# AsherBond/0-kno-vectorx

Hardware: AMD Instinct MI355X
Metric: header_range_256 proofs/sec (higher is better)
Workload: dtype u64 (Goldilocks) / u8 (hashes)

## Files before the change

### 0-kno-vectorx_amd/csrc/poseidon.cuh

```cuda
#pragma once
#include <utility>
#include "gl.cuh"
#include "poseidon_constants.h"

static __constant__ uint64_t POSEIDON_RC[360] = VX_POSEIDON_RC_FOLDED_INIT;

__device__ __forceinline__ uint64_t poseidon_sbox(uint64_t x) {
    const uint64_t x2 = gl_mul_nc(x, x), x3 = gl_mul_nc(x2, x), x4 = gl_mul_nc(x2, x2);
    return gl_mul_nc(x3, x4);
}

template <class T, class TIn>
__device__ __forceinline__ void poseidon_mds_part(const TIn* x, T* y) {
    T u0[3], u2[3], ur[3], ui[3];
#pragma unroll
    for (int a = 0; a < 3; ++a) {
        const T x0 = (T)x[a], x1 = (T)x[3 + a], x2 = (T)x[6 + a], x3 = (T)x[9 + a];
        const T A = x0 + x2, B = x1 + x3;
        u0[a] = A + B;
        u2[a] = A - B;
        ur[a] = x0 - x2;
        ui[a] = x3 - x1;
    }
    const T s0 = u0[0] + u0[1] + u0[2];
    const T a0[3] = {s0 + u0[2], s0 + u0[0], s0 + u0[1]};
    const T a2[3] = {-u2[0] - 2 * u2[1] + 8 * u2[2], -8 * u2[0] - u2[1] - 2 * u2[2], 2 * u2[0] - 8 * u2[1] - u2[2]};
    T p0r[3], p0i[3], p1r[3], p1i[3], p2r[3], p2i[3];
#pragma unroll
    for (int a = 0; a < 3; ++a) {
        p0r[a] = 2 * ur[a] + ui[a];
        p0i[a] = 2 * ui[a] - ur[a];
        p1r[a] = -4 * ur[a] - ui[a];
        p1i[a] = ur[a] - 4 * ui[a];
        p2r[a] = 16 * ur[a] - ui[a];
        p2i[a] = 16 * ui[a] + ur[a];
    }
    const T r0 = p0r[0] + p2i[1] + p1i[2], i0 = p0i[0] - p2r[1] - p1r[2];
    const T r1 = p1r[0] + p0r[1] + p2i[2], i1 = p1i[0] + p0i[1] - p2r[2];
    const T r2 = p2r[0] + p1r[1] + p0r[2], i2 = p2i[0] + p1i[1] + p0i[2];
    const T rr[3] = {r0, r1, r2}, ii[3] = {i0, i1, i2};
#pragma unroll
    for (int c = 0; c < 3; ++c) {
        const T t = 16 * a0[c], pp = t + a2[c], mm = t - a2[c];
        y[c] = pp + rr[c];
        y[3 + c] = mm - ii[c];
        y[6 + c] = pp - rr[c];
        y[9 + c] = mm + ii[c];
    }
}

#ifndef VX_POSEIDON_FP64
#define VX_POSEIDON_FP64 0
#endif
#if VX_POSEIDON_FP64
struct PoseidonRcSplit {
    uint64_t d[360];
    uint32_t h[360];
};
constexpr PoseidonRcSplit poseidon_rc_split() {
    constexpr uint64_t rc[360] = VX_POSEIDON_RC_FOLDED_INIT;
    PoseidonRcSplit t{};
    for (int i = 0; i < 360; ++i) {
        t.d[i] = 0x4330000000000000ULL + (rc[i] & ((1ULL << 43) - 1));
        t.h[i] = (uint32_t)(rc[i] >> 43);
    }
    return t;
}
static __constant__ PoseidonRcSplit POSEIDON_RCT = poseidon_rc_split();
template <int RC>
__device__ __forceinline__ void poseidon_mds(uint64_t* s, int rc_next) {
    constexpr double TWO52 = 4503599627370496.0;
    double xl[12];
    uint32_t xh[12];
#pragma unroll
    for (int i = 0; i < 12; ++i) {
        const uint32_t lo = (uint32_t)s[i], hi = (uint32_t)(s[i] >> 32);
        xl[i] = __longlong_as_double((long long)(((uint64_t)(0x43300000u | (hi & 0x7FFu)) << 32) | lo)) - TWO52;
        xh[i] = hi >> 11;
    }
    double yl[12];
    int32_t yh[12];
    poseidon_mds_part<double>(xl, yl);
    poseidon_mds_part<int32_t>(xh, yh);
    yl[0] += xl[0] * (double)VX_POSEIDON_MDS_DIAG0;
    yh[0] += (int32_t)(xh[0] * VX_POSEIDON_MDS_DIAG0);
#pragma unroll
    for (int r = 0; r < 12; ++r) {
        double magic = TWO52;
        uint32_t ah = (uint32_t)yh[r];
        if (RC == 12 || (RC == 1 && r == 0)) {
            magic = __longlong_as_double((long long)POSEIDON_RCT.d[rc_next + r]);
            ah += POSEIDON_RCT.h[rc_next + r];
        }
        const uint64_t al = (uint64_t)__double_as_longlong(yl[r] + magic) & ((1ULL << 52) - 1);
        const uint64_t w = (uint64_t)(ah >> 21) * GL_EPS + al;
        uint32_t yhi;
        const bool carry = __builtin_add_overflow((uint32_t)(w >> 32), ah << 11, &yhi);
        const uint64_t y = ((uint64_t)yhi << 32) | (uint32_t)w;
        s[r] = y + (carry ? (uint64_t)GL_EPS : 0);
    }
}
#else
template <int RC>
__device__ __forceinline__ void poseidon_mds(uint64_t* s, int rc_next) {
    constexpr uint64_t M52 = (1ULL << 52) - 1;
    uint64_t xl[12];
    uint32_t xh[12];
#pragma unroll
    for (int i = 0; i < 12; ++i) {
        xl[i] = s[i] & M52;
        xh[i] = (uint32_t)(s[i] >> 52);
    }
    int64_t yl[12];
    int32_t yh[12];
    poseidon_mds_part<int64_t>(xl, yl);
    poseidon_mds_part<int32_t>(xh, yh);
    yl[0] += (int64_t)(xl[0] * VX_POSEIDON_MDS_DIAG0);
    yh[0] += (int32_t)(xh[0] * VX_POSEIDON_MDS_DIAG0);
#pragma unroll
    for (int r = 0; r < 12; ++r) {
        uint64_t al = (uint64_t)yl[r];
        uint32_t ah = (uint32_t)yh[r];
        if (RC == 12 || (RC == 1 && r == 0)) {
            const uint64_t c = POSEIDON_RC[rc_next + r];
            al += c & M52;
            ah += (uint32_t)(c >> 52);
        }
        const uint64_t w = (uint64_t)(ah >> 12) * GL_EPS + al;
        uint32_t yhi;
        const bool carry = __builtin_add_overflow((uint32_t)(w >> 32), ah << 20, &yhi);
        const uint64_t y = ((uint64_t)yhi << 32) | (uint32_t)w;
        s[r] = y + (carry ? (uint64_t)GL_EPS : 0);
    }
}

#endif

#ifndef VX_POSEIDON_SPLIT_PARTIAL
#define VX_POSEIDON_SPLIT_PARTIAL 1
#endif
__device__ __forceinline__ uint64_t poseidon_mds_split(uint64_t s0, uint64_t* xl, uint32_t* xh, int rc_next) {
    constexpr uint64_t M52 = (1ULL << 52) - 1;
    xl[0] = s0 & M52;
    xh[0] = (uint32_t)(s0 >> 52);
    int64_t yl[12];
    int32_t yh[12];
    poseidon_mds_part<int64_t>(xl, yl);
    poseidon_mds_part<int32_t>(xh, yh);
    yl[0] += (int64_t)(xl[0] * VX_POSEIDON_MDS_DIAG0);
    yh[0] += (int32_t)(xh[0] * VX_POSEIDON_MDS_DIAG0);
#pragma unroll
    for (int r = 1; r < 12; ++r) {
        const uint64_t al = (uint64_t)yl[r];
        const uint32_t hh = (uint32_t)yh[r] + (uint32_t)(al >> 52);
        xh[r] = hh & 0xFFFu;
        xl[r] = (uint64_t)(hh >> 12) * GL_EPS + (al & M52);
    }
    const uint64_t c = POSEIDON_RC[rc_next];
    const uint64_t al = (uint64_t)yl[0] + (c & M52);
    const uint32_t ah = (uint32_t)yh[0] + (uint32_t)(c >> 52);
    const uint64_t w = (uint64_t)(ah >> 12) * GL_EPS + al;
    uint32_t yhi;
    const bool carry = __builtin_add_overflow((uint32_t)(w >> 32), ah << 20, &yhi);
    const uint64_t y = ((uint64_t)yhi << 32) | (uint32_t)w;
    return y + (carry ? (uint64_t)GL_EPS : 0);
}
__device__ __forceinline__ void poseidon_mds_split_out(uint64_t s0, uint64_t* xl, uint32_t* xh, uint64_t* s, int rc_next) {
    constexpr uint64_t M52 = (1ULL << 52) - 1;
    xl[0] = s0 & M52;
    xh[0] = (uint32_t)(s0 >> 52);
    int64_t yl[12];
    int32_t yh[12];
    poseidon_mds_part<int64_t>(xl, yl);
    poseidon_mds_part<int32_t>(xh, yh);
    yl[0] += (int64_t)(xl[0] * VX_POSEIDON_MDS_DIAG0);
    yh[0] += (int32_t)(xh[0] * VX_POSEIDON_MDS_DIAG0);
#pragma unroll
    for (int r = 0; r < 12; ++r) {
        const uint64_t c = POSEIDON_RC[rc_next + r];
        const uint64_t al = (uint64_t)yl[r] + (c & M52);
        const uint32_t ah = (uint32_t)yh[r] + (uint32_t)(c >> 52);
        const uint64_t w = (uint64_t)(ah >> 12) * GL_EPS + al;
        uint32_t yhi;
        const bool carry = __builtin_add_overflow((uint32_t)(w >> 32), ah << 20, &yhi);
        const uint64_t y = ((uint64_t)yhi << 32) | (uint32_t)w;
        s[r] = y + (carry ? (uint64_t)GL_EPS : 0);
    }
}

template <bool CANON = true>
__device__ __forceinline__ void poseidon_permute(uint64_t* s) {
    int rc = 12;
#pragma unroll
    for (int i = 0; i < 12; ++i) s[i] = gl_add_nc(s[i], POSEIDON_RC[i]);
#pragma unroll 1
    for (int r = 0; r < 3; ++r) {
#pragma unroll
        for (int i = 0; i < 12; ++i) s[i] = poseidon_sbox(s[i]);
        poseidon_mds<12>(s, rc);
        rc += 12;
    }
#pragma unroll
    for (int i = 0; i < 12; ++i) s[i] = poseidon_sbox(s[i]);
    poseidon_mds<1>(s, rc);
    rc += 12;
#if VX_POSEIDON_SPLIT_PARTIAL && !VX_POSEIDON_FP64
    {
        constexpr uint64_t M52 = (1ULL << 52) - 1;
        uint64_t xl[12];
        uint32_t xh[12];
#pragma unroll
        for (int i = 1; i < 12; ++i) {
            xl[i] = s[i] & M52;
            xh[i] = (uint32_t)(s[i] >> 52);
        }
        uint64_t s0 = s[0];
#pragma unroll 1
        for (int r = 0; r < 21; ++r) {
            s0 = poseidon_mds_split(poseidon_sbox(s0), xl, xh, rc);
            rc += 12;
        }
        poseidon_mds_split_out(poseidon_sbox(s0), xl, xh, s, rc);
        rc += 12;
    }
#else
#pragma unroll 1
    for (int r = 0; r < 21; ++r) {
        s[0] = poseidon_sbox(s[0]);
        poseidon_mds<1>(s, rc);
        rc += 12;
    }
    s[0] = poseidon_sbox(s[0]);
    poseidon_mds<12>(s, rc);
    rc += 12;
#endif
#pragma unroll 1
    for (int r = 0; r < 3; ++r) {
#pragma unroll
        for (int i = 0; i < 12; ++i) s[i] = poseidon_sbox(s[i]);
        poseidon_mds<12>(s, rc);
        rc += 12;
    }
#pragma unroll
    for (int i = 0; i < 12; ++i) s[i] = poseidon_sbox(s[i]);
    poseidon_mds<0>(s, 0);
    if (CANON) {
#pragma unroll
        for (int i = 0; i < 12; ++i) s[i] = gl_canon(s[i]);
    }
}

__device__ __forceinline__ uint64_t poseidon_mds_coop(uint64_t s, int l, uint64_t* g) {
    constexpr uint32_t C[12] = VX_POSEIDON_MDS_CIRC_INIT;
    if (l < 12) g[l] = s;
    __builtin_amdgcn_fence(__ATOMIC_RELEASE, "wavefront");
    __builtin_amdgcn_wave_barrier();
    __builtin_amdgcn_fence(__ATOMIC_ACQUIRE, "wavefront");
    uint64_t al = 0, ah = 0;
    const int r = l < 12 ? l : 0;
#pragma unroll
    for (int i = 0; i < 12; ++i) {
        int j = r + i;
        if (j >= 12) j -= 12;
        const uint64_t x = g[j];
        al += (uint64_t)(uint32_t)x * C[i];
        ah += (x >> 32) * C[i];
    }
    if (l == 0) {
        const uint64_t x0 = g[0];
        al += (uint64_t)(uint32_t)x0 * VX_POSEIDON_MDS_DIAG0;
        ah += (x0 >> 32) * VX_POSEIDON_MDS_DIAG0;
    }
    __builtin_amdgcn_fence(__ATOMIC_RELEASE, "wavefront");
    __builtin_amdgcn_wave_barrier();
    __builtin_amdgcn_fence(__ATOMIC_ACQUIRE, "wavefront");
    const uint64_t w = (ah >> 32) * GL_EPS + al;
    uint32_t yhi;
    const bool carry = __builtin_add_overflow((uint32_t)(w >> 32), (uint32_t)ah, &yhi);
    const uint64_t y = ((uint64_t)yhi << 32) | (uint32_t)w;
    return y + (carry ? (uint64_t)GL_EPS : 0);
}
#ifndef VX_POSEIDON_COOP_DPP
#define VX_POSEIDON_COOP_DPP 1
#endif
template <int N>
__device__ __forceinline__ uint32_t dpp_ror(uint32_t x) {
    return (uint32_t)__builtin_amdgcn_update_dpp(0, (int)x, 0x120 + N, 0xf, 0xf, false);
}
struct CoopCoef {
    uint32_t c[16];
};
static __device__ const uint32_t POSEIDON_MDS_CIRC_DEV[12] = VX_POSEIDON_MDS_CIRC_INIT;
template <int N>
__device__ __forceinline__ void coop_coef_one(CoopCoef& k, int l) {
    const int q = (int)dpp_ror<N>((uint32_t)l);
    int d = q - l;
    if (d < 0) d += 12;
    k.c[N] = (q < 12 && l < 12) ? POSEIDON_MDS_CIRC_DEV[d < 12 ? d : 0] : 0;
}
template <int... Ns>
__device__ __forceinline__ void coop_coef_all(CoopCoef& k, int l, std::integer_sequence<int, Ns...>) {
    (coop_coef_one<Ns + 1>(k, l), ...);
}
template <int N>
__device__ __forceinline__ void coop_mac_one(const CoopCoef& k, uint64_t s, uint64_t& al, uint64_t& ah) {
    const uint32_t lo = dpp_ror<N>((uint32_t)s), hi = dpp_ror<N>((uint32_t)(s >> 32));
    al += (uint64_t)lo * k.c[N];
    ah += (uint64_t)hi * k.c[N];
}
template <int... Ns>
__device__ __forceinline__ void coop_mac_all(const CoopCoef& k, uint64_t s, uint64_t& al, uint64_t& ah, std::integer_sequence<int, Ns...>) {
    (coop_mac_one<Ns + 1>(k, s, al, ah), ...);
}
__device__ __forceinline__ uint64_t poseidon_mds_coop_dpp(uint64_t s, int l, const CoopCoef& k) {
    uint64_t al = (uint64_t)(uint32_t)s * k.c[0], ah = (s >> 32) * k.c[0];
    coop_mac_all(k, s, al, ah, std::make_integer_sequence<int, 15>{});
    if (l == 0) {
        al += (uint64_t)(uint32_t)s * VX_POSEIDON_MDS_DIAG0;
        ah += (s >> 32) * VX_POSEIDON_MDS_DIAG0;
    }
    const uint64_t w = (ah >> 32) * GL_EPS + al;
    uint32_t yhi;
    const bool carry = __builtin_add_overflow((uint32_t)(w >> 32), (uint32_t)ah, &yhi);
    const uint64_t y = ((uint64_t)yhi << 32) | (uint32_t)w;
    return y + (carry ? (uint64_t)GL_EPS : 0);
}
template <bool CANON = true>
__device__ __forceinline__ uint64_t poseidon_permute_coop(uint64_t s, int l, uint64_t* g) {
    const int lc = l < 12 ? l : 0;
#if VX_POSEIDON_COOP_DPP
    CoopCoef k;
    k.c[0] = l < 12 ? POSEIDON_MDS_CIRC_DEV[0] : 0;
    coop_coef_all(k, l, std::make_integer_sequence<int, 15>{});
    if (l >= 12) s = 0;
#pragma unroll 1
    for (int r = 0; r < 30; ++r) {
        s = gl_add_nc(s, POSEIDON_RC[12 * r + lc]);
        const bool full = r < 4 || r >= 26;
        if (full || l == 0) s = poseidon_sbox(s);
        s = poseidon_mds_coop_dpp(s, l, k);
    }
    return CANON ? gl_canon(s) : s;
#endif
#pragma unroll 1
    for (int r = 0; r < 30; ++r) {
        s = gl_add_nc(s, POSEIDON_RC[12 * r + lc]);
        const bool full = r < 4 || r >= 26;
        if (full || l == 0) s = poseidon_sbox(s);
        s = poseidon_mds_coop(s, l, g);
    }
    return CANON ? gl_canon(s) : s;
}
```

Measured before the change: 9.035.

## Keep Poseidon partial-round state in frequency domain across rounds

Replaces the 22 partial Poseidon rounds with a version that holds the 12-element state in a transformed (FFT-like) split 48/16-bit integer representation. Each round computes only the new element 0 and updates the transformed state incrementally, normalising lazily, with a single transform on entry and exit. This aims to cut the per-round MDS cost. In exchange it adds complex bound-dependent arithmetic that can overflow if the bounds are wrong, plus extra register pressure. It is enabled by default through a macro.

After: 9.508, median of 6. 1.05x the previous value.

```diff
diff --git a/0-kno-vectorx_amd/csrc/poseidon.cuh b/0-kno-vectorx_amd/csrc/poseidon.cuh
--- a/0-kno-vectorx_amd/csrc/poseidon.cuh
+++ b/0-kno-vectorx_amd/csrc/poseidon.cuh
@@ -188,20 +188,35 @@
     }
 }
 
-template <bool CANON = true>
-__device__ __forceinline__ void poseidon_permute(uint64_t* s) {
-    int rc = 12;
-#pragma unroll
-    for (int i = 0; i < 12; ++i) s[i] = gl_add_nc(s[i], POSEIDON_RC[i]);
-#pragma unroll 1
-    for (int r = 0; r < 3; ++r) {
-#pragma unroll
-        for (int i = 0; i < 12; ++i) s[i] = poseidon_sbox(s[i]);
-        poseidon_mds<12>(s, rc);
-        rc += 12;
-    }
-#pragma unroll
-    for (int i = 0; i < 12; ++i) s[i] = poseidon_sbox(s[i]);
+#ifndef VX_POSEIDON_FREQ_PARTIAL
+#define VX_POSEIDON_FREQ_PARTIAL 1
+#endif
+#if VX_POSEIDON_FREQ_PARTIAL
+#include "poseidon_freq.h"
+__device__ __forceinline__ void poseidon_partial_freq(uint64_t* s, int rc) {
+    pfreq::State u;
+    pfreq::enter(s, u);
+    uint64_t x0 = s[0];
+#pragma unroll 1
+    for (int r = 0; r < 11; ++r) {
+        uint64_t y0 = pfreq::round_y0(u, x0);
+        uint64_t t = poseidon_sbox(gl_add_nc(y0, POSEIDON_RC[rc]));
+        pfreq::round_put<false>(u, x0, y0, t);
+        x0 = t;
+        y0 = pfreq::round_y0(u, x0);
+        t = poseidon_sbox(gl_add_nc(y0, POSEIDON_RC[rc + 12]));
+        pfreq::round_put<true>(u, x0, y0, t);
+        x0 = t;
+        rc += 24;
+    }
+    pfreq::leave(u, x0, &POSEIDON_RC[rc], s);
+}
+#endif
+
+__device__ __forceinline__ void poseidon_partial_rounds(uint64_t* s, int rc) {
+#if VX_POSEIDON_FREQ_PARTIAL
+    poseidon_partial_freq(s, rc);
+#else
     poseidon_mds<1>(s, rc);
     rc += 12;
 #if VX_POSEIDON_SPLIT_PARTIAL && !VX_POSEIDON_FP64
@@ -221,7 +236,6 @@
             rc += 12;
         }
         poseidon_mds_split_out(poseidon_sbox(s0), xl, xh, s, rc);
-        rc += 12;
     }
 #else
 #pragma unroll 1
@@ -232,8 +246,26 @@
     }
     s[0] = poseidon_sbox(s[0]);
     poseidon_mds<12>(s, rc);
-    rc += 12;
-#endif
+#endif
+#endif
+}
+
+template <bool CANON = true>
+__device__ __forceinline__ void poseidon_permute(uint64_t* s) {
+    int rc = 12;
+#pragma unroll
+    for (int i = 0; i < 12; ++i) s[i] = gl_add_nc(s[i], POSEIDON_RC[i]);
+#pragma unroll 1
+    for (int r = 0; r < 3; ++r) {
+#pragma unroll
+        for (int i = 0; i < 12; ++i) s[i] = poseidon_sbox(s[i]);
+        poseidon_mds<12>(s, rc);
+        rc += 12;
+    }
+#pragma unroll
+    for (int i = 0; i < 12; ++i) s[i] = poseidon_sbox(s[i]);
+    poseidon_partial_rounds(s, rc);
+    rc += 12 * 23;
 #pragma unroll 1
     for (int r = 0; r < 3; ++r) {
 #pragma unroll
diff --git a/0-kno-vectorx_amd/csrc/poseidon_freq.h b/0-kno-vectorx_amd/csrc/poseidon_freq.h
--- /dev/null
+++ b/0-kno-vectorx_amd/csrc/poseidon_freq.h
@@ -0,0 +1,172 @@
+#pragma once
+#include <stdint.h>
+
+#if defined(__HIP_DEVICE_COMPILE__)
+#define PFREQ_FN __device__ __forceinline__
+#elif defined(__HIPCC__)
+#define PFREQ_FN __host__ __device__ inline
+#else
+#define PFREQ_FN static inline
+#endif
+#if defined(__clang__)
+#define PFREQ_UNROLL _Pragma("unroll")
+#else
+#define PFREQ_UNROLL
+#endif
+
+namespace pfreq {
+
+constexpr int LB = 48, HB = 16;
+constexpr uint64_t ML = (1ULL << LB) - 1;
+constexpr uint64_t EPS = 0xFFFFFFFFULL;
+constexpr uint64_t KL = (ML + 1 - EPS) << 12;
+constexpr uint32_t KH = ((1u << HB) - 1) << 12;
+constexpr int64_t BOUND_L = 4322LL << LB;
+constexpr int32_t BOUND_H = 4322 << HB;
+constexpr int64_t BOUND_YL = 3307LL << LB;
+constexpr int32_t BOUND_YH = 3307 << HB;
+
+struct State {
+    int64_t l[12];
+    int32_t h[12];
+};
+
+PFREQ_FN void keep(int64_t& x) {
+#if defined(__HIP_DEVICE_COMPILE__)
+    asm("" : "+v"(x));
+#else
+    (void)x;
+#endif
+}
+PFREQ_FN void keep(int32_t&) {}
+PFREQ_FN int32_t minus_one() {
+    int32_t k = -1;
+#if defined(__HIP_DEVICE_COMPILE__)
+    asm("" : "+s"(k));
+#endif
+    return k;
+}
+
+template <class T, class TIn>
+PFREQ_FN void fft_in(const TIn* x, T* u) {
+PFREQ_UNROLL
+    for (int a = 0; a < 3; ++a) {
+        const T x0 = (T)x[a], x1 = (T)x[3 + a], x2 = (T)x[6 + a], x3 = (T)x[9 + a];
+        const T A = x0 + x2, B = x1 + x3;
+        u[a] = A + B;
+        u[3 + a] = A - B;
+        u[6 + a] = x0 - x2;
+        u[9 + a] = x3 - x1;
+    }
+}
+
+template <class T>
+PFREQ_FN void block(const T* u, T* a) {
+    const T *u0 = u, *u2 = u + 3, *ur = u + 6, *ui = u + 9;
+    const T s0 = u0[0] + u0[1] + u0[2];
+    a[0] = s0 + u0[2], a[1] = s0 + u0[0], a[2] = s0 + u0[1];
+    T P, N;
+#define PFREQ_PN(i, pos, neg) P = pos, N = neg, keep(P), keep(N), a[i] = P - N, keep(a[i])
+    PFREQ_PN(3, 8 * u2[2], 2 * u2[1] + u2[0]);
+    PFREQ_PN(4, 0, 8 * u2[0] + 2 * u2[2] + u2[1]);
+    PFREQ_PN(5, 2 * u2[0], 8 * u2[1] + u2[2]);
+    PFREQ_PN(6, 16 * ui[1] + 2 * ur[0] + ui[0] + ur[1] + ur[2], 4 * ui[2]);
+    PFREQ_PN(9, 4 * ur[2] + 2 * ui[0] + ui[1] + ui[2], 16 * ur[1] + ur[0]);
+    PFREQ_PN(7, 16 * ui[2] + 2 * ur[1] + ui[1] + ur[2], 4 * ur[0] + ui[0]);
+    PFREQ_PN(10, 2 * ui[1] + ur[0] + ui[2], 16 * ur[2] + 4 * ui[0] + ur[1]);
+    PFREQ_PN(8, 16 * ur[0] + 2 * ur[2] + ui[2], 4 * ur[1] + ui[0] + ui[1]);
+    PFREQ_PN(11, 16 * ui[0] + 2 * ui[2] + ur[0] + ur[1], 4 * ui[1] + ur[2]);
+#undef PFREQ_PN
+    keep(a[0]), keep(a[1]), keep(a[2]);
+}
+
+PFREQ_FN uint64_t join(uint64_t l, uint32_t h) {
+    const uint64_t w = (uint64_t)(h >> HB) * EPS + l;
+    uint32_t yhi;
+    const bool carry = __builtin_add_overflow((uint32_t)(w >> 32), h << (32 - HB), &yhi);
+    const uint64_t y = ((uint64_t)yhi << 32) | (uint32_t)w;
+    return y + (carry ? EPS : 0);
+}
+
+PFREQ_FN void normalise(int64_t& l, int32_t& h) {
+    const int32_t hh = h + (int32_t)(l >> LB);
+    const int32_t u = hh >> HB;
+    h = hh & (int32_t)((1u << HB) - 1);
+    const uint32_t mhi = ((uint32_t)((uint64_t)l >> 32) & (uint32_t)(ML >> 32)) + (uint32_t)u;
+    l = (int64_t)(((uint64_t)mhi << 32) | (uint32_t)l) + (int64_t)u * (int64_t)minus_one();
+}
+
+PFREQ_FN void enter(const uint64_t* s, State& u) {
+    uint64_t xl[12];
+    uint32_t xh[12];
+PFREQ_UNROLL
+    for (int i = 0; i < 12; ++i) {
+        xl[i] = s[i] & ML;
+        xh[i] = (uint32_t)(s[i] >> LB);
+    }
+    fft_in<int64_t>(xl, u.l);
+    fft_in<int32_t>(xh, u.h);
+}
+
+PFREQ_FN uint64_t round_y0(State& u, uint64_t x0) {
+    int64_t al[12];
+    int32_t ah[12];
+    block<int64_t>(u.l, al);
+    block<int32_t>(u.h, ah);
+    const int64_t yl = 16 * al[0] + al[3] + al[6] + 8 * (int64_t)(x0 & ML);
+    const int32_t yh = 16 * ah[0] + ah[3] + ah[6] + 8 * (int32_t)(x0 >> LB);
+#ifdef PFREQ_TRACK_Y
+    PFREQ_TRACK_Y(yl, yh);
+#endif
+PFREQ_UNROLL
+    for (int c = 0; c < 3; ++c) {
+        u.l[c] = 64 * al[c], u.h[c] = 64 * ah[c];
+        u.l[3 + c] = 4 * al[3 + c], u.h[3 + c] = 4 * ah[3 + c];
+        u.l[6 + c] = 2 * al[6 + c], u.h[6 + c] = 2 * ah[6 + c];
+        u.l[9 + c] = 2 * al[9 + c], u.h[9 + c] = 2 * ah[9 + c];
+    }
+    return join((uint64_t)yl + KL, (uint32_t)yh + KH);
+}
+template <bool ALL>
+PFREQ_FN void round_put(State& u, uint64_t x0, uint64_t y0, uint64_t t) {
+    const int64_t el = 8 * (int64_t)(x0 & ML) + (int64_t)(t & ML) - (int64_t)(y0 & ML);
+    const int32_t eh = 8 * (int32_t)(x0 >> LB) + (int32_t)(t >> LB) - (int32_t)(y0 >> LB);
+    u.l[0] += el, u.l[3] += el, u.l[6] += el;
+    u.h[0] += eh, u.h[3] += eh, u.h[6] += eh;
+#ifdef PFREQ_TRACK
+PFREQ_UNROLL
+    for (int i = 0; i < 12; ++i) PFREQ_TRACK(u.l[i], u.h[i]);
+#endif
+PFREQ_UNROLL
+    for (int i = 0; i < (ALL ? 12 : 3); ++i) normalise(u.l[i], u.h[i]);
+PFREQ_UNROLL
+    for (int i = 0; i < 12; ++i) keep(u.l[i]);
+}
+
+PFREQ_FN void leave(const State& u, uint64_t x0, const uint64_t* rc, uint64_t* s) {
+    int64_t al[12], yl[12];
+    int32_t ah[12], yh[12];
+    block<int64_t>(u.l, al);
+    block<int32_t>(u.h, ah);
+PFREQ_UNROLL
+    for (int c = 0; c < 3; ++c) {
+        const int64_t tl = 16 * al[c], pl = tl + al[3 + c], ml = tl - al[3 + c];
+        yl[c] = pl + al[6 + c], yl[3 + c] = ml - al[9 + c], yl[6 + c] = pl - al[6 + c], yl[9 + c] = ml + al[9 + c];
+        const int32_t th = 16 * ah[c], ph = th + ah[3 + c], mh = th - ah[3 + c];
+        yh[c] = ph + ah[6 + c], yh[3 + c] = mh - ah[9 + c], yh[6 + c] = ph - ah[6 + c], yh[9 + c] = mh + ah[9 + c];
+    }
+    yl[0] += 8 * (int64_t)(x0 & ML);
+    yh[0] += 8 * (int32_t)(x0 >> LB);
+PFREQ_UNROLL
+    for (int r = 0; r < 12; ++r) {
+        const uint64_t c = rc[r];
+        const int64_t vl = yl[r] + (int64_t)(c & ML);
+        const int32_t vh = yh[r] + (int32_t)(c >> LB);
+#ifdef PFREQ_TRACK_Y
+        PFREQ_TRACK_Y(vl, vh);
+#endif
+        s[r] = join((uint64_t)vl + KL, (uint32_t)vh + KH);
+    }
+}
+
+}
```
